# lazear/sage

Measured on AMD Instinct MI355X. Metric: spectra/sec (whole node), fragment-index search-and-score, human tryptic narrow search, higher is better.
Workload: dtype f32

## Files before the change

### include/sage_hip.h

```cpp
#ifndef SAGE_HIP_H
#define SAGE_HIP_H

#include <stddef.h>
#include <stdint.h>

#ifdef __cplusplus
extern "C" {
#endif

#define SAGE_HIP_ABI_VERSION 6

enum {
    SAGE_HIP_OK = 0,
    SAGE_HIP_ERR_INVALID = 1,
    SAGE_HIP_ERR_NO_DEVICE = 2,
    SAGE_HIP_ERR_HIP = 3,
    SAGE_HIP_ERR_UNSUPPORTED = 4,
    SAGE_HIP_ERR_OOM = 5,
    SAGE_HIP_ERR_INTERNAL = 6
};

enum { SAGE_TOL_PPM = 0, SAGE_TOL_PCT = 1, SAGE_TOL_DA = 2 };
typedef struct SageTolerance {
    int32_t kind;
// ... 174 lines not shown
typedef struct SageTiming {
    float prelim_ms;
    float rescore_ms;
    float total_ms;
    uint32_t n_launches;
    uint32_t n_wide;
    uint32_t arena_entries;
    uint32_t n_retry;
    float retry_ms;
    uint32_t n_tied;
    uint32_t n_ways;
} SageTiming;
int sage_hip_last_timing(const SageScorer* scorer, SageTiming* out);
int sage_hip_scorer_set_timing_interval(SageScorer* scorer, uint32_t every);

int sage_hip_host_alloc(uint64_t bytes, void** out);
void sage_hip_host_free(void* p);

int sage_hip_debug_phase_cycles(SageScorer* scorer, unsigned long long* out32);
int sage_hip_debug_prune_counters(SageScorer* scorer, unsigned long long* out4);
int sage_hip_debug_filter_counters(SageScorer* scorer, unsigned long long* out4);
int sage_hip_debug_heavy_counters(SageScorer* scorer, unsigned long long* out2);
int sage_hip_debug_heavy_routes(SageScorer* scorer, unsigned long long* out2);
int sage_hip_debug_handover_route(SageScorer* scorer, uint32_t* out);
#define SAGE_HIP_RESCORE_INST_CHIMERA 1u
#define SAGE_HIP_RESCORE_INST_KINDS2 2u
#define SAGE_HIP_RESCORE_INST_FAST 4u
#define SAGE_HIP_RESCORE_INST_ACC 8u
#define SAGE_HIP_RESCORE_INST_PROF 16u
#define SAGE_HIP_RESCORE_INST_BIG 32u
#define SAGE_HIP_RESCORE_INST_NONE 0xFFFFFFFFu
int sage_hip_debug_rescore_instance(SageScorer* scorer, uint32_t* out);

typedef struct SageDbLayout {
    uint64_t np, nf;
    uint32_t tile_shift, n_tiles, lut_stride;
    float lut_scale;
    uint32_t tile2_shift, n_tiles2, lut2_stride;
    float lut2_scale;
    uint32_t lut2_words;
    uint32_t pep_lut_bins;
    float pep_lut_inv_w;
    uint32_t ion_lo_bits, ion_hi_bits;
    uint32_t max_ions, max_len;
    uint64_t tm2_pos_len;
} SageDbLayout;
// ... 388 lines not shown
```

### sage_amd/_lib.py

```python
import ctypes as C
import os

import numpy as np

from . import build as _build

c_float_p = C.POINTER(C.c_float)
c_u8_p = C.POINTER(C.c_uint8)
c_u32_p = C.POINTER(C.c_uint32)
c_u64_p = C.POINTER(C.c_uint64)


class SageTolerance(C.Structure):
    _fields_ = [("kind", C.c_int32), ("lo", C.c_float), ("hi", C.c_float)]


class SageTheoretical(C.Structure):
    _fields_ = [("peptide_index", C.c_uint32), ("fragment_mz", C.c_float)]


class SageDbParams(C.Structure):
    _fields_ = [
        ("bucket_size", C.c_uint64),
        ("missed_cleavages", C.c_int32),
# ... 344 lines not shown
        "sage_hip_scorer_destroy": (None, [vp]),
        "sage_hip_scorer_clone": (C.c_int, [vp, C.POINTER(vp)]),
        "sage_hip_score_batch": (C.c_int, [vp, C.POINTER(SageSpectrumBatch), vp, c_u32_p]),
        "sage_hip_batch_upload": (C.c_int, [vp, C.POINTER(SageSpectrumBatch), C.POINTER(vp)]),
        "sage_hip_batch_free": (None, [vp]),
        "sage_hip_batch_process_upload": (C.c_int, [vp, C.POINTER(SageRawBatch), C.c_uint64, C.c_int, C.c_float, C.c_uint32,
                                                    C.POINTER(vp), c_u32_p]),
        "sage_hip_batch_download": (C.c_int, [vp, c_u64_p, c_float_p, c_float_p, c_float_p]),
        "sage_hip_batch_upload_kinds": (C.c_int, [vp, C.POINTER(SageSpectrumBatch), c_u8_p, C.POINTER(vp)]),
        "sage_hip_batch_process_upload_kinds": (C.c_int, [vp, C.POINTER(SageRawBatch), c_u8_p, C.c_uint64, C.c_int, C.c_float,
                                                          C.c_uint32, C.POINTER(vp), c_u32_p]),
        "sage_hip_score_batch_kinds": (C.c_int, [vp, C.POINTER(SageSpectrumBatch), c_u8_p, vp, c_u32_p]),
        "sage_hip_score_resident": (C.c_int, [vp, vp, vp, c_u32_p]),
        "sage_hip_initial_hits": (C.c_int, [vp, vp, c_u64_p, C.c_uint32, c_u32_p, c_u64_p, c_u64_p]),
        "sage_hip_last_timing": (C.c_int, [vp, C.POINTER(SageTiming)]),
        "sage_hip_scorer_set_timing_interval": (C.c_int, [vp, C.c_uint32]),
        "sage_hip_annotate_resident": (C.c_int, [vp, vp, vp, c_u32_p, C.POINTER(SageFragments)]),
        "sage_hip_quick_score_resident": (C.c_int, [vp, vp, C.c_int, c_u8_p]),
        "sage_hip_debug_phase_cycles": (C.c_int, [vp, c_u64_p]),
        "sage_hip_debug_prune_counters": (C.c_int, [vp, c_u64_p]),
        "sage_hip_debug_filter_counters": (C.c_int, [vp, c_u64_p]),
        "sage_hip_debug_heavy_counters": (C.c_int, [vp, c_u64_p]),
        "sage_hip_debug_heavy_routes": (C.c_int, [vp, c_u64_p]),
        "sage_hip_debug_handover_route": (C.c_int, [vp, c_u32_p]),
        "sage_hip_debug_rescore_instance": (C.c_int, [vp, c_u32_p]),
        "sage_hip_debug_db_layout": (C.c_int, [vp, C.POINTER(SageDbLayout)]),
        "sage_hip_debug_db_table": (C.c_int, [vp, C.c_int, vp, C.c_uint64, c_u64_p]),
        "sage_hip_host_alloc": (C.c_int, [C.c_uint64, C.POINTER(vp)]),
        "sage_hip_host_free": (None, [vp]),
        "sage_hip_rescore": (C.c_int, [C.c_int, C.POINTER(SageRescoreInput), C.POINTER(SageRescoreOutput)]),
        "sage_hip_hostdb_competition_keys": (C.c_int, [vp, c_u32_p, C.c_uint64, c_u32_p, c_u32_p, c_u32_p, c_u32_p]),
        "sage_hip_predict_rt": (C.c_int, [C.c_int, C.POINTER(SageRtInput), C.POINTER(SageRtOutput)]),
        "sage_hip_hostdb_feature_peptides": (C.c_int, [vp, c_u32_p, C.c_uint64, c_u64_p, c_u8_p, c_float_p]),
        "sage_hip_mzml_read": (C.c_int, [C.c_char_p, C.c_uint32, C.c_int, C.POINTER(vp)]),
        "sage_hip_mzml_view": (C.c_int, [vp, C.POINTER(SageRawBatch)]),
        "sage_hip_mzml_check_searchable": (C.c_int, [vp]),
        "sage_hip_mzml_spectrum_id": (C.c_char_p, [vp, C.c_uint64]),
        "sage_hip_mzml_free": (None, [vp]),
        "sage_hip_mzml_read_sn": (C.c_int, [C.c_char_p, C.c_uint32, C.c_int, C.c_int, C.POINTER(vp)]),
        "sage_hip_mzml_ion_injection_time": (C.c_float, [vp, C.c_uint64]),
        "sage_hip_mzml_precursor_ref": (C.c_char_p, [vp, C.c_uint64]),
        "sage_hip_mgf_read": (C.c_int, [C.c_char_p, C.c_uint32, C.POINTER(vp)]),
        "sage_hip_mzml_isolation_kinds": (C.c_int, [vp, c_u8_p]),
        "sage_hip_mzml_charge_zero": (C.c_int, [vp, c_u8_p]),
        "sage_hip_parse_f32": (C.c_int, [C.c_char_p, C.c_uint64, c_float_p]),
        "sage_hip_tmt": (C.c_int, [C.c_int, C.POINTER(SageTmtInput), C.POINTER(SageTmtOutput)]),
# ... 32 lines not shown
        "sage_hip_write_protein_lfq": (C.c_int, [C.c_char_p, C.POINTER(C.c_char_p), C.c_uint32, c_u32_p, C.c_uint32,
                                                 C.POINTER(SageProteinLfqOutput), C.POINTER(C.c_char_p), C.c_uint32]),
        "sage_hip_tmt_rollup": (C.c_int, [C.c_int, C.POINTER(SageTmtRollupInput), C.POINTER(SageTmtRollupOutput)]),
        "sage_hip_write_tmt_rollup": (C.c_int, [C.c_char_p, C.c_char_p, C.POINTER(C.c_char_p), C.c_uint32, C.c_uint64, C.POINTER(C.c_char_p),
                                                c_u32_p, c_u32_p, c_u32_p, C.POINTER(C.c_double)]),
        "sage_hip_precursor_purity": (C.c_int, [C.c_int, C.POINTER(SagePurityInput), C.POINTER(SagePurityOutput)]),
        "sage_hip_write_purity": (C.c_int, [C.c_char_p, C.c_uint64, c_u64_p, c_u32_p, C.POINTER(C.c_char_p), c_u8_p, C.POINTER(C.c_char_p),
                                            c_float_p, c_float_p, C.POINTER(SagePurityOutput), C.POINTER(C.c_char_p), C.c_uint32]),
    }
    for name, (res, args) in sig.items():
        fn = getattr(lib, name)
        fn.restype = res
        fn.argtypes = args
    _lib = lib
    return lib


EXPORTED_SYMBOLS = [
    "sage_hip_last_error", "sage_hip_abi_version", "sage_hip_hostdb_build", "sage_hip_hostdb_free",
    "sage_hip_hostdb_view", "sage_hip_hostdb_peptide_string", "sage_hip_hostdb_peptide_proteins",
    "sage_hip_hostdb_peptide_info", "sage_hip_process_ms2", "sage_hip_device_count", "sage_hip_db_create", "sage_hip_db_destroy",
    "sage_hip_db_device_bytes", "sage_hip_scorer_create", "sage_hip_scorer_destroy", "sage_hip_scorer_clone", "sage_hip_score_batch",
    "sage_hip_batch_upload", "sage_hip_batch_free", "sage_hip_batch_process_upload", "sage_hip_batch_download", "sage_hip_score_resident", "sage_hip_initial_hits",
    "sage_hip_last_timing", "sage_hip_scorer_set_timing_interval", "sage_hip_annotate_resident", "sage_hip_quick_score_resident", "sage_hip_debug_phase_cycles", "sage_hip_debug_prune_counters", "sage_hip_debug_filter_counters", "sage_hip_debug_heavy_counters", "sage_hip_debug_heavy_routes", "sage_hip_debug_handover_route", "sage_hip_debug_rescore_instance", "sage_hip_debug_db_layout", "sage_hip_debug_db_table", "sage_hip_host_alloc", "sage_hip_host_free",
    "sage_hip_rescore", "sage_hip_hostdb_competition_keys", "sage_hip_fasta_num_targets", "sage_hip_prefilter_chunk_size",
    "sage_hip_hostdb_build_chunk", "sage_hip_hostdb_merge_kept", "sage_hip_predict_rt", "sage_hip_hostdb_feature_peptides",
    "sage_hip_write_results", "sage_hip_mzml_read", "sage_hip_mzml_view", "sage_hip_mzml_check_searchable", "sage_hip_mzml_spectrum_id", "sage_hip_mzml_free",
    "sage_hip_lfq", "sage_hip_write_lfq", "sage_hip_mzml_read_sn", "sage_hip_mzml_ion_injection_time", "sage_hip_mzml_precursor_ref",
    "sage_hip_tmt", "sage_hip_write_tmt", "sage_hip_mgf_read", "sage_hip_mzml_isolation_kinds", "sage_hip_mzml_charge_zero",
    "sage_hip_parse_f32", "sage_hip_batch_upload_kinds", "sage_hip_batch_process_upload_kinds", "sage_hip_score_batch_kinds",
    "sage_hip_lfq_im", "sage_hip_mzml_mobility", "sage_hip_mzml_has_mobility",
    "sage_hip_protein_groups", "sage_hip_group_string", "sage_hip_group_strings_free", "sage_hip_group_graph_build",
    "sage_hip_group_graph_view", "sage_hip_group_graph_free", "sage_hip_hostdb_protein_name", "sage_hip_write_results_grouped",
    "sage_hip_hostdb_isomer_groups", "sage_hip_score_candidates_resident", "sage_hip_last_candidates_timing",
    "sage_hip_localise_resident", "sage_hip_ascore_from_counts", "sage_hip_last_localise_timing",
    "sage_hip_protein_lfq", "sage_hip_write_protein_lfq",
    "sage_hip_precursor_purity", "sage_hip_write_purity",
    "sage_hip_tmt_rollup", "sage_hip_write_tmt_rollup",
]


def check(rc):
    if rc != 0:
        msg = load().sage_hip_last_error()
        raise SageHipError(f"libsage_hip status {rc}: {msg.decode() if msg else ''}")


# ... 3 lines not shown
```

### sage_amd/csrc/capi.hip

```cpp
#include <algorithm>
#include <chrono>
#include <future>

#include "capi_state.h"
#include "crlog.h"

extern "C" {

static uint32_t scorer_tol_mode(const sagecore::Tol& t, uint32_t ion_lo_bits, uint32_t ion_hi_bits) {
    uint32_t mode = 0;
    if (t.kind == 0 && t.lo == -t.hi) mode |= sagecore::TOL_SYM;
    if (ion_lo_bits > ion_hi_bits) return mode;
    float ion_lo, ion_hi;
    std::memcpy(&ion_lo, &ion_lo_bits, 4);
    std::memcpy(&ion_hi, &ion_hi_bits, 4);
    const double lo = sagecore::FAST_DIV_LO, hi = sagecore::FAST_DIV_HI;
    bool ok = ion_lo >= lo && ion_hi <= hi;
    if (ok && t.kind == 0)
        for (const float b : {t.lo, t.hi}) {
            const double a = std::fabs((double)b);
            ok = ok && a > 0.0 && (double)ion_lo / 255.0 * a >= 2.0 * lo && (double)ion_hi * a <= 0.5 * hi;
        }
    if (ok) mode |= sagecore::TOL_FAST;
    return mode;
// ... 1402 lines not shown
    for (size_t b = 0; b < DBG_BLOCKS; b++)
        for (int k = 0; k < 32; k++) out32[k] += all[b * 32 + k];
    return SAGE_HIP_OK;
}

static int sum_dbg_words(SageScorer* s, uint32_t first_word, uint32_t count, unsigned long long* out) {
    if (!s || !out) return fail(SAGE_HIP_ERR_INVALID, "null argument");
    if (!s->dbg.p) return fail(SAGE_HIP_ERR_INVALID, "set SAGE_HIP_PHASE_CLOCKS=1 before creating the scorer");
    std::vector<unsigned long long> all((size_t)DBG_BLOCKS * DBG_PRUNE_WORDS);
    HIP_TRY(hipMemcpy(all.data(), s->dbg.p + (size_t)DBG_BLOCKS * 32, all.size() * 8, hipMemcpyDeviceToHost));
    for (uint32_t k = 0; k < count; k++) out[k] = 0;
    for (size_t b = 0; b < DBG_BLOCKS; b++)
        for (uint32_t k = 0; k < count; k++) out[k] += all[b * DBG_PRUNE_WORDS + first_word + k];
    return SAGE_HIP_OK;
}

int sage_hip_debug_prune_counters(SageScorer* s, unsigned long long* out4) { return sum_dbg_words(s, 0, 4, out4); }
int sage_hip_debug_filter_counters(SageScorer* s, unsigned long long* out4) { return sum_dbg_words(s, 4, 4, out4); }

int sage_hip_debug_heavy_counters(SageScorer* s, unsigned long long* out2) { return sum_dbg_words(s, 8, 2, out2); }

int sage_hip_debug_heavy_routes(SageScorer* s, unsigned long long* out2) { return sum_dbg_words(s, 10, 2, out2); }

int sage_hip_debug_handover_route(SageScorer* s, uint32_t* out) {
    if (!s || !out) return fail(SAGE_HIP_ERR_INVALID, "null argument");
    *out = s->last_hand ? 1u : 0u;
    return SAGE_HIP_OK;
}

int sage_hip_debug_rescore_instance(SageScorer* s, uint32_t* out) {
    if (!s || !out) return fail(SAGE_HIP_ERR_INVALID, "null argument");
    static_assert(RESCORE_INST_CHIMERA == SAGE_HIP_RESCORE_INST_CHIMERA && RESCORE_INST_KINDS2 == SAGE_HIP_RESCORE_INST_KINDS2 &&
                      RESCORE_INST_FAST == SAGE_HIP_RESCORE_INST_FAST && RESCORE_INST_ACC == SAGE_HIP_RESCORE_INST_ACC &&
                      RESCORE_INST_PROF == SAGE_HIP_RESCORE_INST_PROF && RESCORE_INST_BIG == SAGE_HIP_RESCORE_INST_BIG &&
                      RESCORE_INST_NONE == SAGE_HIP_RESCORE_INST_NONE,
                  "include/sage_hip.h names the bits of device_types.h");
    *out = s->last_rescore;
    return SAGE_HIP_OK;
}


int sage_hip_host_alloc(uint64_t bytes, void** out) {
    if (!out) return fail(SAGE_HIP_ERR_INVALID, "null argument");
    HIP_TRY(hipHostMalloc(out, bytes ? bytes : 1, hipHostMallocDefault));
    if (void* d = device_view(*out)) {
        std::lock_guard<std::mutex> lock(g_blocks_mu);
// ... 53 lines not shown
```

### sage_amd/csrc/core.h

```cpp
#pragma once
#include <stdint.h>

#if defined(__HIPCC__)
#define SAGE_HD __host__ __device__ __forceinline__
#else
#define SAGE_HD inline
#endif

namespace sagecore {

constexpr float PROTON = 1.0072764f;
constexpr float NEUTRON = 1.00335f;

struct Tol {
    int kind;
    float lo, hi;
};

SAGE_HD void tol_bounds(const Tol& t, float center, float& out_lo, float& out_hi) {
    if (t.kind == 0) {
        float dlo = center * t.lo / 1000000.0f;
        float dhi = center * t.hi / 1000000.0f;
        out_lo = center + dlo;
        out_hi = center + dhi;
// ... 432 lines not shown
}
SAGE_HD KindSeg kind_seg_next(const KindSeg& g, uint32_t lm1) {
    const uint32_t lo = g.lo + g.len;
    const uint32_t len = lm1 < 64u - lo ? lm1 : 64u - lo;
    return KindSeg{lo, len, 0u, g.kind + 1u};
}
SAGE_HD uint64_t kind_seg_mask(const KindSeg& g) { return g.len >= 64u ? ~0ull : ((1ull << g.len) - 1ull) << (g.lo & 63u); }

SAGE_HD uint32_t kinds2_bound(uint32_t j0, uint32_t lm1) { return j0 >= lm1 ? 0u : lm1 - j0 < 64u ? lm1 - j0 : 64u; }
SAGE_HD uint64_t kinds2_nt_mask(uint32_t bound) { return bound >= 64u ? ~0ull : (1ull << bound) - 1ull; }
SAGE_HD uint32_t kinds2_idx0_c(uint32_t j0, uint32_t lm1) { return j0 >= lm1 ? j0 - lm1 : 0u; }
SAGE_HD uint32_t kinds2_decode(uint32_t j, uint32_t lm1, bool& cterm) {
    cterm = j >= lm1;
    return j - (cterm ? lm1 : 0u);
}

constexpr uint32_t COOP_ITEMS_CAP = 64;
SAGE_HD uint32_t coop_items_below(uint64_t M1, uint64_t M2, uint64_t M3, uint32_t i) {
    const uint64_t below = i >= 64u ? ~0ull : (1ull << i) - 1ull;
    return (uint32_t)(__builtin_popcountll(M1 & below) + __builtin_popcountll(M2 & below) + __builtin_popcountll(M3 & below));
}
SAGE_HD uint32_t coop_item_pos(uint64_t M1, uint64_t M2, uint64_t M3, uint32_t i, uint32_t c) {
    return coop_items_below(M1, M2, M3, i) + (c >= 2u ? (uint32_t)((M1 >> i) & 1ull) : 0u) + (c >= 3u ? (uint32_t)((M2 >> i) & 1ull) : 0u);
}

struct Score {
    uint32_t peptide;
    uint32_t matched_b, matched_y;
    float summed_b, summed_y;
    uint32_t longest_b, longest_y;
    float ppm_difference;
    uint32_t precursor_charge;
    int isotope_error;
};

SAGE_HD void score_candidate(Score& s, const float* ions, uint32_t lm1, const uint8_t* ion_kinds, uint32_t n_kinds,
                             uint32_t max_fc, const float* masses, const float* intensities, uint32_t n_peaks,
                             const Tol& fragment_tol) {
    Run b_run = {0, 0, 0, 0}, y_run = {0, 0, 0, 0};
    s.matched_b = s.matched_y = 0;
    s.summed_b = s.summed_y = 0.0f;
    s.ppm_difference = 0.0f;
    for (uint32_t k = 0; k < n_kinds; k++) {
        const bool nterm_kind = ion_kinds[k] <= 2;
        const float* series = ions + (uint64_t)k * lm1;
        for (uint32_t idx = 0; idx < lm1; idx++) {
// ... 180 lines not shown
```

### sage_amd/csrc/device_types.h

```cpp
#pragma once
#include <stdint.h>

#include <string>

#include "../../include/sage_hip.h"
#include "core.h"

namespace sagehip {

struct DevDbView {
    const float* pep_mono;
    uint32_t np;
    const uint32_t* pep_lut;
    uint32_t pep_lut_bins;
    float pep_lut_inv_w;
    const SageTheoretical* pm_frag;
    const uint64_t* pm_off;
    const float* ions;
    const uint64_t* ion_off;
    const uint32_t* pep_info;
    const SageTheoretical* tm_frag;
    const uint32_t* tm_lut;
    uint32_t tile_shift;
    uint32_t n_tiles;
    uint32_t lut_stride;
    float lut_scale;
    const SageTheoretical* tm2_frag;
    const sagecore::LutWord* tm2_l1;
    const uint32_t* tm2_pos;
    uint32_t lut2_words;
    uint32_t tile2_shift;
    uint32_t n_tiles2;
    uint32_t lut2_stride;
    float lut2_scale;
    uint64_t nf;
    uint8_t ion_kinds[8];
    uint32_t n_kinds;
};

constexpr uint32_t TILE_SHIFT_MAX = 15;
__host__ __device__ inline size_t tm_lut_index(uint32_t t, uint32_t c, uint32_t lut_stride) { return (size_t)t * lut_stride + c; }

constexpr uint32_t DBG_BLOCKS = 4096, DBG_PRUNE_WORDS = 12;
constexpr size_t DBG_TOTAL_WORDS = (size_t)DBG_BLOCKS * (32 + DBG_PRUNE_WORDS);

struct DevScorer {
    sagecore::Tol precursor_tol, fragment_tol;
    sagecore::PbmReach pbm_reach;
    uint32_t min_matched_peaks;
    int min_isotope_err, max_isotope_err;
    uint32_t min_precursor_charge, max_precursor_charge;
    uint32_t override_precursor_charge;
    int max_fragment_charge;
    uint32_t chimera;
    uint32_t report_psms;
    uint32_t wide_window;
    int score_type;
    uint32_t kmax;
    uint32_t big_path;
    uint32_t long_runs;
    uint32_t tol_mode;
    uint32_t list_cap;
    uint32_t wcap;
    uint32_t dbg_flags;
    uint32_t prune_min;
    uint32_t rescore_general;
// ... 208 lines not shown
```

### sage_amd/csrc/kernels.hip

```cpp
#include <hip/hip_runtime.h>

#include <type_traits>

#include "crlog.h"
#include "device_types.h"

using namespace sagecore;

namespace sagehip {

namespace {

#ifndef SAGE_PRELIM_WAVES
#define SAGE_PRELIM_WAVES 5
#endif
#ifndef SAGE_RESCORE_WAVES
#define SAGE_RESCORE_WAVES 5
#endif
#ifndef SAGE_NARROW_WAVES
#define SAGE_NARROW_WAVES 5
#endif
#ifndef SAGE_PROBE_PER_LANE
#define SAGE_PROBE_PER_LANE 2
#endif
// ... 29 lines not shown
#if SAGE_PRELIM_WAVES
#define SAGE_PRELIM_WAVES_ATTR __attribute__((amdgpu_waves_per_eu(SAGE_PRELIM_WAVES, SAGE_PRELIM_WAVES)))
#else
#define SAGE_PRELIM_WAVES_ATTR
#endif
#if SAGE_RESCORE_WAVES
#define SAGE_RESCORE_WAVES_ATTR __attribute__((amdgpu_waves_per_eu(SAGE_RESCORE_WAVES, SAGE_RESCORE_WAVES)))
#else
#define SAGE_RESCORE_WAVES_ATTR
#endif

constexpr uint32_t WAVE = 64;
constexpr uint32_t NO_WINDOW = 0xFFFFFFFFu;
constexpr uint32_t FAST_TIE_WORDS = PBM_WORDS + PLUT_BINS;
constexpr uint32_t CNT_ROW_HEADER = 4;
constexpr uint32_t PROBE_BATCH_WORDS = SAGE_PROBE_PER_LANE * 64;
constexpr uint32_t PROBE_TCS_WORDS = PROBE_BATCH_WORDS <= 64 ? 64 : PROBE_BATCH_WORDS <= 128 ? 128 : PROBE_BATCH_WORDS <= 256 ? 256 : 512;
constexpr uint32_t PROBE_TABLE_WORDS = 4 * PROBE_BATCH_WORDS + PROBE_TCS_WORDS;

enum { DBG_PRUNE_CAND = 0, DBG_PRUNE_ITEMS = 1, DBG_PRUNE_EARLY = 2, DBG_PRUNE_MIXED = 3 };
enum { DBG_FILTER_FLAT_CHUNKS = 4, DBG_FILTER_FLAT_TRIPS = 5, DBG_FILTER_FLAT_WOULD = 6, DBG_FILTER_LANE_TRIPS = 7 };
enum { DBG_HEAVY_CHUNKS = 8, DBG_HEAVY_ITEMS = 9 };
enum { DBG_HEAVY_ONE_TRIP = 10, DBG_HEAVY_PER_CHARGE = 11 };
enum { DBG_NARROW_LUT = 26, DBG_NARROW_CELLS = 27, DBG_RESCORE = 28, DBG_TILE_LUT = 29, DBG_TILE_CELLS = 30, DBG_TILE_CAND = 31 };
struct PhaseClock {
    unsigned long long* slot;
    long long t;
    __device__ __forceinline__ void bytes(int which, unsigned long long n) {
        if (slot) atomicAdd(&slot[which - row_base], n);
    }
    int row_base;
    unsigned long long* prune;
    uint32_t pruned_here;
    __device__ __forceinline__ void pruned(uint64_t lanes, uint32_t items) {
        if (slot && lanes) {
            pruned_here += (uint32_t)__popcll(lanes);
            if ((threadIdx.x & 63u) == 0) {
                atomicAdd(&prune[DBG_PRUNE_CAND], (unsigned long long)__popcll(lanes));
                atomicAdd(&prune[DBG_PRUNE_ITEMS], (unsigned long long)items);
            }
        }
    }
    __device__ __forceinline__ void filter_trips(bool flat, uint32_t flat_trips, uint32_t lane_trips) {
        if (slot && (threadIdx.x & 63u) == 0) {
            if (flat) {
                atomicAdd(&prune[DBG_FILTER_FLAT_CHUNKS], 1ull);
                atomicAdd(&prune[DBG_FILTER_FLAT_TRIPS], (unsigned long long)flat_trips);
                atomicAdd(&prune[DBG_FILTER_FLAT_WOULD], (unsigned long long)lane_trips);
            } else {
                atomicAdd(&prune[DBG_FILTER_LANE_TRIPS], (unsigned long long)lane_trips);
            }
        }
    }
    __device__ __forceinline__ void heavy(uint32_t items) {
        if (slot && (threadIdx.x & 63u) == 0) {
            atomicAdd(&prune[DBG_HEAVY_CHUNKS], 1ull);
            atomicAdd(&prune[DBG_HEAVY_ITEMS], (unsigned long long)items);
        }
    }
    __device__ __forceinline__ void heavy_route(bool one_trip) {
        if (slot && (threadIdx.x & 63u) == 0) atomicAdd(&prune[one_trip ? DBG_HEAVY_ONE_TRIP : DBG_HEAVY_PER_CHARGE], 1ull);
    }
    __device__ __forceinline__ void prune_outcome(bool left_early, bool any_pass) {
        if (slot && (threadIdx.x & 63u) == 0) {
            if (left_early) atomicAdd(&prune[DBG_PRUNE_EARLY], 1ull);
            else if (any_pass && pruned_here) atomicAdd(&prune[DBG_PRUNE_MIXED], 1ull);
        }
        pruned_here = 0;
    }
    __device__ __forceinline__ void start(unsigned long long* dbg, uint32_t blk, uint32_t kernel) {
        slot = dbg ? dbg + (size_t)(blk % DBG_BLOCKS) * 32 + kernel * 8 : nullptr;
        row_base = (int)kernel * 8;
        prune = dbg ? dbg + (size_t)DBG_BLOCKS * 32 + (size_t)(blk % DBG_BLOCKS) * DBG_PRUNE_WORDS : nullptr;
        pruned_here = 0;
        if (slot) t = clock64();
    }
    __device__ __forceinline__ void mark(int phase) {
        if (slot) {
            const long long n = clock64();
            if ((threadIdx.x & 63u) == 0) atomicAdd(&slot[phase], (unsigned long long)(n - t));
            t = n;
        }
    }
    __device__ __forceinline__ void rebase(uint32_t kernel) {
        if (slot) slot += (int)kernel * 8 - row_base;
        row_base = (int)kernel * 8;
    }
};

struct NoClock {
    static constexpr unsigned long long* slot = nullptr;
    __device__ __forceinline__ void bytes(int, unsigned long long) {}
    __device__ __forceinline__ void pruned(uint64_t, uint32_t) {}
    __device__ __forceinline__ void prune_outcome(bool, bool) {}
    __device__ __forceinline__ void filter_trips(bool, uint32_t, uint32_t) {}
    __device__ __forceinline__ void heavy(uint32_t) {}
    __device__ __forceinline__ void heavy_route(bool) {}
    __device__ __forceinline__ void start(unsigned long long*, uint32_t, uint32_t) {}
    __device__ __forceinline__ void mark(int) {}
    __device__ __forceinline__ void rebase(uint32_t) {}
};

__device__ __forceinline__ uint32_t lane_id() { return threadIdx.x & 63u; }

constexpr uint32_t N_XCD = 8;
__device__ __forceinline__ uint32_t xcd_position_fwd(uint32_t b, uint32_t n, uint32_t chunk) {
    if (chunk == 0) return b;
    const uint32_t group = N_XCD * chunk;
    if (b >= n / group * group) return b;
    const uint32_t x = b % N_XCD, i = b / N_XCD;
    return ((i / chunk) * N_XCD + x) * chunk + i % chunk;
}
__device__ __forceinline__ uint32_t xcd_position(uint32_t b, uint32_t n, uint32_t chunk) {
    const uint32_t p = xcd_position_fwd(b, n, chunk & 0x7FFFFFFFu);
    return (chunk & 0x80000000u) ? n - 1 - p : p;
}

__device__ __forceinline__ uint32_t fresh_zero() {
    uint32_t z;
    asm volatile("v_mov_b32 %0, 0" : "=v"(z));
// ... 2374 lines not shown
}
__device__ __forceinline__ uint8_t* rescore_flat_area(const float* pm, const float* pi) { return (uint8_t*)(pi + (pi - pm)); }
__device__ __forceinline__ RescoreLds carve_rescore(unsigned char* scratch, unsigned char* fixed, const DevBatchView& b) {
    RescoreLds l;
    l.pbm = (uint32_t*)scratch;
    l.plut = l.pbm + PBM_WORDS;
    l.s_sorted = (double*)l.pbm;
    l.s_key = (long long*)(l.s_sorted + 64);
    l.qkeys = (QuickKey*)(l.plut + PLUT_BINS);
    l.hdr = (uint32_t*)fixed;
    l.meta = (uint2*)(fixed + RESCORE_HDR_WORDS * 4);
    l.pm = (float*)(fixed + RESCORE_HEAD_BYTES);
    l.pi = l.pm + b.pcap;
    l.rm = rescore_flat_area(l.pm, l.pi);
    l.rm2 = l.rm + b.pcap;
    l.stage = (uint32_t*)(fixed + RESCORE_HEAD_BYTES + (size_t)b.pcap * 8 + rescore_flat_bytes(b.pcap));
    return l;
}

__device__ __forceinline__ uint32_t lane_run(uint32_t v, uint32_t src_lane) { return (uint32_t)__builtin_amdgcn_readlane((int)v, (int)src_lane); }
__device__ __forceinline__ uint64_t lane_run(uint64_t v, uint32_t src_lane) { return lane_value(v, src_lane); }
constexpr uint32_t DENSE_CAP = 384;
static_assert(DENSE_CAP % 64 == 0 && DENSE_CAP * 10 + DENSE_CAP / 8 <= PBM_WORDS * 4, "the dense work list fits the bitmap");
template <class PC, bool LONG = false, bool FAST = false, bool FLAT = !LONG, bool KINDS2 = false>
__device__ __forceinline__ void score_candidates(const DevDbView& db, const DevScorer& sc, const uint32_t* pbm, const uint32_t* plut,
                                                 const float* pm, const float* pi, const uint32_t P, const float inv_w,
                                                 const bool valid, const uint64_t ion_base, const uint32_t lm1, const uint32_t nfz,
                                                 const bool any_fz2, const bool any_fz3, const uint32_t nterm_mask, const bool sym_tol,
                                                 Score& s, PC& pc, const bool dense_ok = false) {
    static_assert(!(FLAT && LONG), "the flat route's worker offsets and tags are those of the one-register instances");
    const bool flat_ok = FLAT && !(sc.dbg_flags & 8192u);
    const uint32_t lane = lane_id();
    typedef typename std::conditional<LONG, uint64_t, uint32_t>::type RunReg;
    constexpr bool DENSE = !LONG;
    RunReg b_run = 0, y_run = 0;
    uint32_t mm = 0;
    const bool scored = valid && lm1 && nfz;
    const float* __restrict__ my = db.ions + ion_base;
    const uint32_t nions = scored ? (KINDS2 ? 2u : db.n_kinds) * lm1 : 0u;
    for (uint32_t j0 = 0; __ballot(j0 < nions) != 0ull; j0 += 64u) {
        const bool act = j0 < nions;
        const uint32_t n_here = !act ? 0u : nions - j0 < 64u ? nions - j0 : 64u;
        uint64_t m1 = 0, m2 = 0, m3 = 0;
        bool flat = false;
        uint32_t flat_trips = 0;
        if (flat_ok) {
            uint8_t* const flat_area = rescore_flat_area(pm, pi);
            const uint32_t flat_cap = rescore_flat_bytes((uint32_t)(pi - pm));
            const uint32_t cnt = act && nfz <= 3u ? flat_octets(n_here) : 0u;
            const uint32_t incl = wave_incl_scan_dpp(cnt), start = incl - cnt;
            const uint32_t T = (uint32_t)__builtin_amdgcn_readlane((int)incl, 63);
            const uint32_t stride = flat_stride(T);
            if (T != 0u && flat_area_bytes(T, 1u + (any_fz2 ? 1u : 0u) + (any_fz3 ? 1u : 0u)) <= flat_cap &&
                (__ballot(cnt > flat_route_bar(T)) != 0ull || (sc.dbg_flags & 16384u))) {
                flat = true;
                uint8_t* const a1 = flat_area;
                uint8_t* const a2 = a1 + stride;
                uint8_t* const a3 = a2 + (any_fz2 ? stride : 0u);
                for (uint32_t k = 0; __ballot(k < cnt) != 0ull; k++)
                    if (k < cnt) a1[start + k] = (uint8_t)lane;
                lds_sync();
                const uint64_t ion_at = flat_item_base(ion_base + j0, start);
                for (uint32_t base = 0; base < T; base += WAVE) {
                    const uint32_t t = base + lane;
                    const bool on = t < T;
                    const uint32_t src = (on ? (uint32_t)a1[t] : 0u) << 2;
                    const uint64_t ib = ((uint64_t)(uint32_t)__builtin_amdgcn_ds_bpermute((int)src, (int)(uint32_t)(ion_at >> 32)) << 32) |
                                        (uint32_t)__builtin_amdgcn_ds_bpermute((int)src, (int)(uint32_t)ion_at);
                    if (on) {
                        const float* __restrict__ q = db.ions + flat_item_ion(ib, t);
                        const float i0 = q[0], i1 = q[1], i2 = q[2], i3 = q[3], i4 = q[4], i5 = q[5], i6 = q[6], i7 = q[7];
                        const uint32_t x0 = pbm_index(i0), x1 = pbm_index(i1), x2 = pbm_index(i2), x3 = pbm_index(i3);
                        const uint32_t x4 = pbm_index(i4), x5 = pbm_index(i5), x6 = pbm_index(i6), x7 = pbm_index(i7);
#define SAGE_FLAT_BYTE(F)                                                                                             \
    (uint8_t)(pbm_bit(F(x0)) | (pbm_bit(F(x1)) << 1) | (pbm_bit(F(x2)) << 2) | (pbm_bit(F(x3)) << 3) | (pbm_bit(F(x4)) << 4) | \
              (pbm_bit(F(x5)) << 5) | (pbm_bit(F(x6)) << 6) | (pbm_bit(F(x7)) << 7))
#define SAGE_FLAT_C1(X) (X)
#define SAGE_FLAT_C2(X) ((X) >> 1)
#define SAGE_FLAT_C3(X) (__umulhi((X), 0xAAAAAAABu) >> 1)
                        a1[t] = SAGE_FLAT_BYTE(SAGE_FLAT_C1);
                        if (any_fz2) a2[t] = SAGE_FLAT_BYTE(SAGE_FLAT_C2);
                        if (any_fz3) a3[t] = SAGE_FLAT_BYTE(SAGE_FLAT_C3);
#undef SAGE_FLAT_C3
#undef SAGE_FLAT_C2
#undef SAGE_FLAT_C1
// ... 8 lines not shown
                        const uint32_t w0 = wp[0], w1 = wp[1], w2 = wp[2];
                        m1 = (uint64_t)flat_mask_word(w0, w1, start) | ((uint64_t)flat_mask_word(w1, w2, start) << 32);
                    }
                    if (any_fz2 && nfz >= 2u) {
                        const uint32_t* const wp = (const uint32_t*)(a2 + at);
                        const uint32_t w0 = wp[0], w1 = wp[1], w2 = wp[2];
                        m2 = (uint64_t)flat_mask_word(w0, w1, start) | ((uint64_t)flat_mask_word(w1, w2, start) << 32);
                    }
                    if (any_fz3 && nfz >= 3u) {
                        const uint32_t* const wp = (const uint32_t*)(a3 + at);
                        const uint32_t w0 = wp[0], w1 = wp[1], w2 = wp[2];
                        m3 = (uint64_t)flat_mask_word(w0, w1, start) | ((uint64_t)flat_mask_word(w1, w2, start) << 32);
                    }
                }
            }
            flat_trips = (T + 63u) / 64u;
        }
        if (pc.slot) {
            uint32_t would = act ? (n_here + 3u) >> 2 : 0u;
            for (int o = 32; o; o >>= 1) { const uint32_t v = (uint32_t)__shfl_xor((int)would, o, 64); would = v > would ? v : would; }
            pc.filter_trips(flat, flat_trips, would);
        }
        if (act && !flat) {
            const float* __restrict__ q = my + j0;
            float n0 = q[0], n1 = q[1], n2 = q[2], n3 = q[3];
            for (uint32_t r = 0; r < n_here; r += 4) {
                const float i0 = n0, i1 = n1, i2 = n2, i3 = n3;
                n0 = q[r + 4]; n1 = q[r + 5]; n2 = q[r + 6]; n3 = q[r + 7];
                const uint32_t x0 = pbm_index(i0), x1 = pbm_index(i1), x2 = pbm_index(i2), x3 = pbm_index(i3);
                const uint32_t t1 = pbm_bit(x0) | (pbm_bit(x1) << 1) | (pbm_bit(x2) << 2) | (pbm_bit(x3) << 3);
                m1 |= (uint64_t)t1 << r;
                if (any_fz2) {
                    const uint32_t t2 = pbm_bit(x0 >> 1) | (pbm_bit(x1 >> 1) << 1) | (pbm_bit(x2 >> 1) << 2) | (pbm_bit(x3 >> 1) << 3);
                    m2 |= (uint64_t)t2 << r;
                }
                if (any_fz3) {
                    const uint32_t t3 = pbm_bit(__umulhi(x0, 0xAAAAAAABu) >> 1) | (pbm_bit(__umulhi(x1, 0xAAAAAAABu) >> 1) << 1) |
                                        (pbm_bit(__umulhi(x2, 0xAAAAAAABu) >> 1) << 2) | (pbm_bit(__umulhi(x3, 0xAAAAAAABu) >> 1) << 3);
                    m3 |= (uint64_t)t3 << r;
                }
            }
        }
        if (act) {
            const uint64_t in_chunk = n_here >= 64u ? ~0ull : (1ull << n_here) - 1ull;
            m1 &= in_chunk;
            m2 = nfz >= 2 ? m2 & in_chunk : 0ull;
            m3 = nfz >= 3 ? m3 & in_chunk : 0ull;
            if (nfz > 3) m1 = m2 = m3 = in_chunk;
        }
        pc.mark(6);
        uint32_t hc = act && nfz <= 3 ? (uint32_t)(__popcll(m1) + __popcll(m2) + __popcll(m3)) : 0u;
        {
            const bool drop = hc != 0u && j0 + 64u >= nions && (mm & 0xFFFFu) + (mm >> 16) + hc < sc.prune_min;
            if (pc.slot) pc.pruned(__ballot(drop), wave_sum(drop ? hc : 0u));
            if (drop) {
                m1 = m2 = m3 = 0ull;
                hc = 0u;
            }
        }
        uint64_t bigs = (sc.dbg_flags & 32u) ? 0ull : __ballot(hc > ((sc.dbg_flags & 32768u) ? 0u : COOP_MIN_HITS));
        if ((uint32_t)__popcll(bigs) > COOP_MAX_LANES && !(sc.dbg_flags & 64u)) bigs = 0ull;
        const bool coop_lds = FLAT && DENSE && dense_ok && !(sc.dbg_flags & 262144u) && __ballot(j0 + 64u < nions) == 0ull;
        while (bigs) {
            const uint32_t L = (uint32_t)__ffsll((long long)bigs) - 1;
            bigs &= bigs - 1;
            const uint64_t M1 = lane_value(m1, L), M2 = lane_value(m2, L), M3 = lane_value(m3, L);
            const uint64_t base_L = lane_value((uint64_t)ion_base, L);
            const uint32_t lm1_L = (uint32_t)__builtin_amdgcn_readlane((int)lm1, (int)L);
            const bool on1 = (M1 >> lane) & 1ull, on2 = (M2 >> lane) & 1ull, on3 = (M3 >> lane) & 1ull;
            float it1 = 0.f, it2 = 0.f, it3 = 0.f, tm1 = 0.f, tm2 = 0.f, tm3 = 0.f;
            bool ok1 = false, ok2 = false, ok3 = false;
            const uint32_t N = (uint32_t)(__popcll(M1) + __popcll(M2) + __popcll(M3));
            const bool one_trip = coop_lds && N <= COOP_ITEMS_CAP;
            if (pc.slot) pc.heavy_route(one_trip);
            float sum_b = 0.f, sum_y = 0.f, sum_p = 0.f;
            if (one_trip) {
                uint32_t* const cD = (uint32_t*)pbm;
                float* const cS = (float*)(cD + 64);
                float ionv = 0.f;
                if (on1 || on2 || on3) ionv = db.ions[base_L + j0 + lane];
                uint64_t NT = 0ull;
                if constexpr (KINDS2) {
                    NT = kinds2_nt_mask(kinds2_bound(j0, lm1_L));
                } else {
                    uint64_t rem = M1 | M2 | M3;
// ... 111 lines not shown
                uint64_t S = anyK & seg;
                if (!S) continue;
                anyK ^= S;
                const bool nterm = (nterm_mask >> g.kind) & 1u;
                u_mm += (uint32_t)(__popcll(K1 & seg) + __popcll(K2 & seg) + __popcll(K3 & seg)) << (nterm ? 0u : 16u);
                if (nterm) run_matched_mask(u_b, S >> g.lo, g.idx0);
                else run_matched_mask(u_y, S >> g.lo, g.idx0);
                if (one_trip) continue;
                float acc = nterm ? u_sb : u_sy;
                SAGE_COOP_ADD(S, acc)
                if (nterm) u_sb = acc;
                else u_sy = acc;
            }
            }
#undef SAGE_COOP_ADD
            if (lane == L) {
                s.summed_b = u_sb; s.summed_y = u_sy; s.ppm_difference = u_pp;
                mm = u_mm;
                b_run = u_b; y_run = u_y;
                m1 = m2 = m3 = 0ull;
            }
        }
        pc.mark(7);
        if (DENSE && dense_ok && !(sc.dbg_flags & 128u) && __ballot(j0 + 64u < nions) == 0ull && __ballot(act && nfz > 3u) == 0ull) {
            const uint32_t hcnt = act ? (uint32_t)(__popcll(m1) + __popcll(m2) + __popcll(m3)) : 0u;
            const uint32_t incl = wave_incl_scan_dpp(hcnt);
            const uint32_t T = (uint32_t)__builtin_amdgcn_readlane((int)incl, 63);
            if (T == 0u) continue;
            if (T <= ((sc.dbg_flags & 256u) ? 64u : DENSE_CAP)) {
                uint32_t* const dW = (uint32_t*)pbm;
                float* const dB = (float*)(dW + DENSE_CAP);
                uint16_t* const dT = (uint16_t*)(dB + DENSE_CAP);
                uint32_t* const dF = (uint32_t*)(dT + DENSE_CAP);
                uint32_t pos = incl - hcnt;
                uint64_t any = m1 | m2 | m3;
                while (any) {
                    const uint32_t bit = (uint32_t)__ffsll((long long)any) - 1;
                    any &= any - 1;
                    uint32_t kind_i = 0, idx = j0 + bit;
                    bool cterm = false;
                    if constexpr (KINDS2) idx = kinds2_decode(idx, lm1, cterm);
                    else while (idx >= lm1) { idx -= lm1; kind_i++; }
                    const uint32_t nt = KINDS2 ? (cterm ? 0u : 1u) : (nterm_mask >> kind_i) & 1u;
                    const uint32_t word = idx | (nt << 15) | (bit << 16) | (lane << 24);
                    if ((m1 >> bit) & 1ull) dW[pos++] = word | (1u << 22);
                    if (any_fz2 && ((m2 >> bit) & 1ull)) dW[pos++] = word | (2u << 22);
                    if (any_fz3 && ((m3 >> bit) & 1ull)) dW[pos++] = word | (3u << 22);
                }
                lds_sync();
                for (uint32_t base = 0; base < T; base += WAVE) {
                    const uint32_t i = base + lane;
                    const uint32_t word = i < T ? dW[i] : 0u;
// ... 1611 lines not shown
```

Baseline: 162.9 million.

## Compute both chunks of two-chunk candidates up front to prune early and reuse dense path

For waves whose candidates have between 65 and 128 ions, the kernel now computes the second 64-ion chunk's match masks before scoring the first, so prune checks can count hits from both chunks and drop hopeless candidates before any scoring. The second chunk's masks are parked in unused regions of the LDS bitmap, which lets the first chunk use the dense and cooperative LDS routes that were previously reserved for the final chunk. This aims to skip scoring work for pruned candidates and avoid the slower per-lane walk. In exchange it adds LDS parking with extra syncs, a smaller dense capacity for the first chunk, and new debug counters.

```diff
diff --git a/include/sage_hip.h b/include/sage_hip.h
--- a/include/sage_hip.h
+++ b/include/sage_hip.h
@@ -220,6 +220,7 @@
 int sage_hip_debug_filter_counters(SageScorer* scorer, unsigned long long* out4);
 int sage_hip_debug_heavy_counters(SageScorer* scorer, unsigned long long* out2);
 int sage_hip_debug_heavy_routes(SageScorer* scorer, unsigned long long* out2);
+int sage_hip_debug_long_counters(SageScorer* scorer, unsigned long long* out4);
 int sage_hip_debug_handover_route(SageScorer* scorer, uint32_t* out);
 #define SAGE_HIP_RESCORE_INST_CHIMERA 1u
 #define SAGE_HIP_RESCORE_INST_KINDS2 2u
diff --git a/sage_amd/_lib.py b/sage_amd/_lib.py
--- a/sage_amd/_lib.py
+++ b/sage_amd/_lib.py
@@ -390,6 +390,7 @@
         "sage_hip_debug_filter_counters": (C.c_int, [vp, c_u64_p]),
         "sage_hip_debug_heavy_counters": (C.c_int, [vp, c_u64_p]),
         "sage_hip_debug_heavy_routes": (C.c_int, [vp, c_u64_p]),
+        "sage_hip_debug_long_counters": (C.c_int, [vp, c_u64_p]),
         "sage_hip_debug_handover_route": (C.c_int, [vp, c_u32_p]),
         "sage_hip_debug_rescore_instance": (C.c_int, [vp, c_u32_p]),
         "sage_hip_debug_db_layout": (C.c_int, [vp, C.POINTER(SageDbLayout)]),
@@ -468,7 +469,7 @@
     "sage_hip_hostdb_peptide_info", "sage_hip_process_ms2", "sage_hip_device_count", "sage_hip_db_create", "sage_hip_db_destroy",
     "sage_hip_db_device_bytes", "sage_hip_scorer_create", "sage_hip_scorer_destroy", "sage_hip_scorer_clone", "sage_hip_score_batch",
     "sage_hip_batch_upload", "sage_hip_batch_free", "sage_hip_batch_process_upload", "sage_hip_batch_download", "sage_hip_score_resident", "sage_hip_initial_hits",
-    "sage_hip_last_timing", "sage_hip_scorer_set_timing_interval", "sage_hip_annotate_resident", "sage_hip_quick_score_resident", "sage_hip_debug_phase_cycles", "sage_hip_debug_prune_counters", "sage_hip_debug_filter_counters", "sage_hip_debug_heavy_counters", "sage_hip_debug_heavy_routes", "sage_hip_debug_handover_route", "sage_hip_debug_rescore_instance", "sage_hip_debug_db_layout", "sage_hip_debug_db_table", "sage_hip_host_alloc", "sage_hip_host_free",
+    "sage_hip_last_timing", "sage_hip_scorer_set_timing_interval", "sage_hip_annotate_resident", "sage_hip_quick_score_resident", "sage_hip_debug_phase_cycles", "sage_hip_debug_prune_counters", "sage_hip_debug_filter_counters", "sage_hip_debug_heavy_counters", "sage_hip_debug_heavy_routes", "sage_hip_debug_long_counters", "sage_hip_debug_handover_route", "sage_hip_debug_rescore_instance", "sage_hip_debug_db_layout", "sage_hip_debug_db_table", "sage_hip_host_alloc", "sage_hip_host_free",
     "sage_hip_rescore", "sage_hip_hostdb_competition_keys", "sage_hip_fasta_num_targets", "sage_hip_prefilter_chunk_size",
     "sage_hip_hostdb_build_chunk", "sage_hip_hostdb_merge_kept", "sage_hip_predict_rt", "sage_hip_hostdb_feature_peptides",
     "sage_hip_write_results", "sage_hip_mzml_read", "sage_hip_mzml_view", "sage_hip_mzml_check_searchable", "sage_hip_mzml_spectrum_id", "sage_hip_mzml_free",
diff --git a/sage_amd/csrc/capi.hip b/sage_amd/csrc/capi.hip
--- a/sage_amd/csrc/capi.hip
+++ b/sage_amd/csrc/capi.hip
@@ -1448,6 +1448,8 @@
 
 int sage_hip_debug_heavy_routes(SageScorer* s, unsigned long long* out2) { return sum_dbg_words(s, 10, 2, out2); }
 
+int sage_hip_debug_long_counters(SageScorer* s, unsigned long long* out4) { return sum_dbg_words(s, 12, 4, out4); }
+
 int sage_hip_debug_handover_route(SageScorer* s, uint32_t* out) {
     if (!s || !out) return fail(SAGE_HIP_ERR_INVALID, "null argument");
     *out = s->last_hand ? 1u : 0u;
diff --git a/sage_amd/csrc/core.h b/sage_amd/csrc/core.h
--- a/sage_amd/csrc/core.h
+++ b/sage_amd/csrc/core.h
@@ -478,6 +478,25 @@
 }
 SAGE_HD uint32_t coop_item_pos(uint64_t M1, uint64_t M2, uint64_t M3, uint32_t i, uint32_t c) {
     return coop_items_below(M1, M2, M3, i) + (c >= 2u ? (uint32_t)((M1 >> i) & 1ull) : 0u) + (c >= 3u ? (uint32_t)((M2 >> i) & 1ull) : 0u);
+}
+
+constexpr uint32_t PARK_DENSE_STRIDE = 384, DENSE_CAP_PARKED = 192, PARK_COOP_BYTES = 1024, PARK_LDS_BYTES = 4096;
+constexpr uint32_t PARK_STRIPE_BYTES = 64 * 4;
+constexpr uint32_t PARK_AT0 = 1024, PARK_AT1 = 1280, PARK_AT2 = 2304, PARK_AT3 = 2560, PARK_AT4 = 2816, PARK_AT5 = 3456;
+static_assert(DENSE_CAP_PARKED % 64 == 0 && DENSE_CAP_PARKED <= PARK_DENSE_STRIDE, "whole trips, inside the full list's arrays");
+static_assert(PARK_AT0 >= PARK_COOP_BYTES && PARK_AT0 >= DENSE_CAP_PARKED * 4, "behind the one-trip route's words and the short list's intensities");
+static_assert(PARK_AT1 == PARK_AT0 + PARK_STRIPE_BYTES && PARK_AT1 + PARK_STRIPE_BYTES <= PARK_DENSE_STRIDE * 4, "two stripes in front of the ppm terms");
+static_assert(PARK_AT2 >= PARK_DENSE_STRIDE * 4 + DENSE_CAP_PARKED * 4 && PARK_AT3 == PARK_AT2 + PARK_STRIPE_BYTES &&
+                  PARK_AT4 == PARK_AT3 + PARK_STRIPE_BYTES && PARK_AT4 + PARK_STRIPE_BYTES <= PARK_DENSE_STRIDE * 8,
+              "three stripes between the short list's ppm terms and the tags");
+static_assert(PARK_AT5 >= PARK_DENSE_STRIDE * 8 + DENSE_CAP_PARKED * 2 && PARK_AT5 + PARK_STRIPE_BYTES <= PARK_DENSE_STRIDE * 10,
+              "one stripe between the short list's tags and the flags");
+static_assert(PARK_DENSE_STRIDE * 10 + PARK_DENSE_STRIDE / 8 <= PARK_LDS_BYTES, "the flags end inside the bitmap");
+SAGE_HD bool prune_two_chunks(uint32_t matched_so_far, uint32_t hits0, uint32_t hits1, uint32_t prune_min) {
+    return hits0 + hits1 != 0u && matched_so_far + hits0 + hits1 < prune_min;
+}
+SAGE_HD uint32_t park_offset(uint32_t stripe, uint32_t lane) {
+    return (stripe == 0u ? PARK_AT0 : stripe == 1u ? PARK_AT1 : stripe == 2u ? PARK_AT2 : stripe == 3u ? PARK_AT3 : stripe == 4u ? PARK_AT4 : PARK_AT5) + 4u * lane;
 }
 
 struct Score {
diff --git a/sage_amd/csrc/device_types.h b/sage_amd/csrc/device_types.h
--- a/sage_amd/csrc/device_types.h
+++ b/sage_amd/csrc/device_types.h
@@ -41,7 +41,7 @@
 constexpr uint32_t TILE_SHIFT_MAX = 15;
 __host__ __device__ inline size_t tm_lut_index(uint32_t t, uint32_t c, uint32_t lut_stride) { return (size_t)t * lut_stride + c; }
 
-constexpr uint32_t DBG_BLOCKS = 4096, DBG_PRUNE_WORDS = 12;
+constexpr uint32_t DBG_BLOCKS = 4096, DBG_PRUNE_WORDS = 16;
 constexpr size_t DBG_TOTAL_WORDS = (size_t)DBG_BLOCKS * (32 + DBG_PRUNE_WORDS);
 
 struct DevScorer {
diff --git a/sage_amd/csrc/kernels.hip b/sage_amd/csrc/kernels.hip
--- a/sage_amd/csrc/kernels.hip
+++ b/sage_amd/csrc/kernels.hip
@@ -75,6 +75,7 @@
 enum { DBG_FILTER_FLAT_CHUNKS = 4, DBG_FILTER_FLAT_TRIPS = 5, DBG_FILTER_FLAT_WOULD = 6, DBG_FILTER_LANE_TRIPS = 7 };
 enum { DBG_HEAVY_CHUNKS = 8, DBG_HEAVY_ITEMS = 9 };
 enum { DBG_HEAVY_ONE_TRIP = 10, DBG_HEAVY_PER_CHARGE = 11 };
+enum { DBG_LONG_ROUNDS = 12, DBG_LONG_PRUNED = 13, DBG_LONG_DENSE = 14, DBG_LONG_WALK = 15 };
 enum { DBG_NARROW_LUT = 26, DBG_NARROW_CELLS = 27, DBG_RESCORE = 28, DBG_TILE_LUT = 29, DBG_TILE_CELLS = 30, DBG_TILE_CAND = 31 };
 struct PhaseClock {
     unsigned long long* slot;
@@ -114,6 +115,9 @@
     __device__ __forceinline__ void heavy_route(bool one_trip) {
         if (slot && (threadIdx.x & 63u) == 0) atomicAdd(&prune[one_trip ? DBG_HEAVY_ONE_TRIP : DBG_HEAVY_PER_CHARGE], 1ull);
     }
+    __device__ __forceinline__ void long_round(int which, uint32_t n) {
+        if (slot && n && (threadIdx.x & 63u) == 0) atomicAdd(&prune[which], (unsigned long long)n);
+    }
     __device__ __forceinline__ void prune_outcome(bool left_early, bool any_pass) {
         if (slot && (threadIdx.x & 63u) == 0) {
             if (left_early) atomicAdd(&prune[DBG_PRUNE_EARLY], 1ull);
@@ -149,6 +153,7 @@
     __device__ __forceinline__ void filter_trips(bool, uint32_t, uint32_t) {}
     __device__ __forceinline__ void heavy(uint32_t) {}
     __device__ __forceinline__ void heavy_route(bool) {}
+    __device__ __forceinline__ void long_round(int, uint32_t) {}
     __device__ __forceinline__ void start(unsigned long long*, uint32_t, uint32_t) {}
     __device__ __forceinline__ void mark(int) {}
     __device__ __forceinline__ void rebase(uint32_t) {}
@@ -2569,6 +2574,8 @@
 __device__ __forceinline__ uint64_t lane_run(uint64_t v, uint32_t src_lane) { return lane_value(v, src_lane); }
 constexpr uint32_t DENSE_CAP = 384;
 static_assert(DENSE_CAP % 64 == 0 && DENSE_CAP * 10 + DENSE_CAP / 8 <= PBM_WORDS * 4, "the dense work list fits the bitmap");
+static_assert(DENSE_CAP == PARK_DENSE_STRIDE && PBM_WORDS * 4 == PARK_LDS_BYTES && COOP_ITEMS_CAP * 16 == PARK_COOP_BYTES,
+              "core.h: park_offset assumes the dense list's strides, the bitmap's bytes and the one-trip route's 64 words + 3 x 64 floats");
 template <class PC, bool LONG = false, bool FAST = false, bool FLAT = !LONG, bool KINDS2 = false>
 __device__ __forceinline__ void score_candidates(const DevDbView& db, const DevScorer& sc, const uint32_t* pbm, const uint32_t* plut,
                                                  const float* pm, const float* pi, const uint32_t P, const float inv_w,
@@ -2585,10 +2592,24 @@
     const bool scored = valid && lm1 && nfz;
     const float* __restrict__ my = db.ions + ion_base;
     const uint32_t nions = scored ? (KINDS2 ? 2u : db.n_kinds) * lm1 : 0u;
+    const bool two = FLAT && DENSE && dense_ok && !(sc.dbg_flags & 524288u) && __ballot(nions > 64u) != 0ull && __ballot(nions > 128u) == 0ull &&
+                     __ballot(scored && nfz > 3u) == 0ull;
+    if (pc.slot && two) pc.long_round(DBG_LONG_ROUNDS, 1u);
     for (uint32_t j0 = 0; __ballot(j0 < nions) != 0ull; j0 += 64u) {
-        const bool act = j0 < nions;
-        const uint32_t n_here = !act ? 0u : nions - j0 < 64u ? nions - j0 : 64u;
+        const bool first_of_two = two && j0 == 0u, second_of_two = two && j0 != 0u;
         uint64_t m1 = 0, m2 = 0, m3 = 0;
+        uint64_t n1 = 0, n2 = 0, n3 = 0;
+        if (second_of_two) {
+            const uint8_t* const pk = (const uint8_t*)pbm;
+            m1 = (uint64_t)*(const uint32_t*)(pk + park_offset(0u, lane)) | ((uint64_t)*(const uint32_t*)(pk + park_offset(1u, lane)) << 32);
+            if (any_fz2) m2 = (uint64_t)*(const uint32_t*)(pk + park_offset(2u, lane)) | ((uint64_t)*(const uint32_t*)(pk + park_offset(3u, lane)) << 32);
+            if (any_fz3) m3 = (uint64_t)*(const uint32_t*)(pk + park_offset(4u, lane)) | ((uint64_t)*(const uint32_t*)(pk + park_offset(5u, lane)) << 32);
+            lds_sync();
+        } else
+        for (uint32_t jf = first_of_two ? 64u : j0;;) {
+        const bool act = jf < nions;
+        const uint32_t n_here = !act ? 0u : nions - jf < 64u ? nions - jf : 64u;
+        m1 = m2 = m3 = 0ull;
         bool flat = false;
         uint32_t flat_trips = 0;
         if (flat_ok) {
@@ -2607,7 +2628,7 @@
                 for (uint32_t k = 0; __ballot(k < cnt) != 0ull; k++)
                     if (k < cnt) a1[start + k] = (uint8_t)lane;
                 lds_sync();
-                const uint64_t ion_at = flat_item_base(ion_base + j0, start);
+                const uint64_t ion_at = flat_item_base(ion_base + jf, start);
                 for (uint32_t base = 0; base < T; base += WAVE) {
                     const uint32_t t = base + lane;
                     const bool on = t < T;
@@ -2662,11 +2683,11 @@
             pc.filter_trips(flat, flat_trips, would);
         }
         if (act && !flat) {
-            const float* __restrict__ q = my + j0;
-            float n0 = q[0], n1 = q[1], n2 = q[2], n3 = q[3];
+            const float* __restrict__ q = my + jf;
+            float nx0 = q[0], nx1 = q[1], nx2 = q[2], nx3 = q[3];
             for (uint32_t r = 0; r < n_here; r += 4) {
-                const float i0 = n0, i1 = n1, i2 = n2, i3 = n3;
-                n0 = q[r + 4]; n1 = q[r + 5]; n2 = q[r + 6]; n3 = q[r + 7];
+                const float i0 = nx0, i1 = nx1, i2 = nx2, i3 = nx3;
+                nx0 = q[r + 4]; nx1 = q[r + 5]; nx2 = q[r + 6]; nx3 = q[r + 7];
                 const uint32_t x0 = pbm_index(i0), x1 = pbm_index(i1), x2 = pbm_index(i2), x3 = pbm_index(i3);
                 const uint32_t t1 = pbm_bit(x0) | (pbm_bit(x1) << 1) | (pbm_bit(x2) << 2) | (pbm_bit(x3) << 3);
                 m1 |= (uint64_t)t1 << r;
@@ -2688,9 +2709,38 @@
             m3 = nfz >= 3 ? m3 & in_chunk : 0ull;
             if (nfz > 3) m1 = m2 = m3 = in_chunk;
         }
+        if (jf == j0) break;
+        n1 = m1; n2 = m2; n3 = m3;
+        jf = j0;
+        }
+        const bool act = j0 < nions;
         pc.mark(6);
         uint32_t hc = act && nfz <= 3 ? (uint32_t)(__popcll(m1) + __popcll(m2) + __popcll(m3)) : 0u;
-        {
+        if (first_of_two) {
+            const uint32_t h_next = (uint32_t)(__popcll(n1) + __popcll(n2) + __popcll(n3));
+            const bool drop = prune_two_chunks((mm & 0xFFFFu) + (mm >> 16), hc, h_next, sc.prune_min);
+            if (pc.slot) {
+                pc.pruned(__ballot(drop), wave_sum(drop ? hc + h_next : 0u));
+                pc.long_round(DBG_LONG_PRUNED, (uint32_t)__popcll(__ballot(drop && nions > 64u)));
+            }
+            if (drop) {
+                m1 = m2 = m3 = 0ull;
+                n1 = n2 = n3 = 0ull;
+                hc = 0u;
+            }
+            uint8_t* const pk = (uint8_t*)pbm;
+            lds_sync();
+            *(uint32_t*)(pk + park_offset(0u, lane)) = (uint32_t)n1;
+            *(uint32_t*)(pk + park_offset(1u, lane)) = (uint32_t)(n1 >> 32);
+            if (any_fz2) {
+                *(uint32_t*)(pk + park_offset(2u, lane)) = (uint32_t)n2;
+                *(uint32_t*)(pk + park_offset(3u, lane)) = (uint32_t)(n2 >> 32);
+            }
+            if (any_fz3) {
+                *(uint32_t*)(pk + park_offset(4u, lane)) = (uint32_t)n3;
+                *(uint32_t*)(pk + park_offset(5u, lane)) = (uint32_t)(n3 >> 32);
+            }
+        } else {
             const bool drop = hc != 0u && j0 + 64u >= nions && (mm & 0xFFFFu) + (mm >> 16) + hc < sc.prune_min;
             if (pc.slot) pc.pruned(__ballot(drop), wave_sum(drop ? hc : 0u));
             if (drop) {
@@ -2700,7 +2750,7 @@
         }
         uint64_t bigs = (sc.dbg_flags & 32u) ? 0ull : __ballot(hc > ((sc.dbg_flags & 32768u) ? 0u : COOP_MIN_HITS));
         if ((uint32_t)__popcll(bigs) > COOP_MAX_LANES && !(sc.dbg_flags & 64u)) bigs = 0ull;
-        const bool coop_lds = FLAT && DENSE && dense_ok && !(sc.dbg_flags & 262144u) && __ballot(j0 + 64u < nions) == 0ull;
+        const bool coop_lds = FLAT && DENSE && dense_ok && !(sc.dbg_flags & 262144u) && (first_of_two || __ballot(j0 + 64u < nions) == 0ull);
         while (bigs) {
             const uint32_t L = (uint32_t)__ffsll((long long)bigs) - 1;
             bigs &= bigs - 1;
@@ -2858,12 +2908,13 @@
             }
         }
         pc.mark(7);
-        if (DENSE && dense_ok && !(sc.dbg_flags & 128u) && __ballot(j0 + 64u < nions) == 0ull && __ballot(act && nfz > 3u) == 0ull) {
+        if (DENSE && dense_ok && !(sc.dbg_flags & 128u) && (first_of_two || __ballot(j0 + 64u < nions) == 0ull) && __ballot(act && nfz > 3u) == 0ull) {
             const uint32_t hcnt = act ? (uint32_t)(__popcll(m1) + __popcll(m2) + __popcll(m3)) : 0u;
             const uint32_t incl = wave_incl_scan_dpp(hcnt);
             const uint32_t T = (uint32_t)__builtin_amdgcn_readlane((int)incl, 63);
             if (T == 0u) continue;
-            if (T <= ((sc.dbg_flags & 256u) ? 64u : DENSE_CAP)) {
+            if (pc.slot && first_of_two) pc.long_round(T <= ((sc.dbg_flags & 256u) ? 64u : DENSE_CAP_PARKED) ? DBG_LONG_DENSE : DBG_LONG_WALK, 1u);
+            if (T <= ((sc.dbg_flags & 256u) ? 64u : first_of_two ? DENSE_CAP_PARKED : DENSE_CAP)) {
                 uint32_t* const dW = (uint32_t*)pbm;
                 float* const dB = (float*)(dW + DENSE_CAP);
                 uint16_t* const dT = (uint16_t*)(dB + DENSE_CAP);
```

Result: no change. 163.7 million, median of 6 (+0.5%).
